# Kudo510/ImageSequenceRegistrationfor6DPoseEstimationLabeling

Measured on AMD Instinct MI355X. Metric: registered images/sec (T-LESS obj 1-like, synthetic) + final Chamfer error, higher is better.
Workload: dtype bf16

## Files before the change

### imagesequenceregistrationfor6dposeestimationlabeling_amd/_capi.py

```python
from __future__ import annotations

import ctypes as C
from pathlib import Path

import torch

import os

_PKG = Path(__file__).resolve().parent
LIB_PATH = Path(os.environ["ISR_HIP_LIB"]) if os.environ.get("ISR_HIP_LIB") else _PKG / "libisr_hip.so"

ISR_OK = 0
ABI_VERSION = 6
DTYPE_BF16 = 0
DTYPE_F32 = 1
DTYPE_BF16_LOG2 = 2
DTYPE_BF16_LOG2_SCREENED = 3
RANSAC_STAGED = 0
RANSAC_SEQUENTIAL = 1
INLIERS_REFIT = 0
INLIERS_RANSAC = 1
FINAL_REFIT = 0
FINAL_EPNP = 1
TUNE = {"nn_path": 0, "nn_filter": 1, "icp_warm": 2, "nn_plan_rq": 3, "nn_plan_blocks": 4,
        "nn_tile_st": 5, "nn_tile_sq": 6, "nn_tile_tb": 7, "ep_wsum_valu": 8, "k1_f32_chain": 9, "k1_split": 10}


class IsrError(RuntimeError):
    pass


_lib = None

_vp = C.c_void_p
_i = C.c_int
_sz = C.c_size_t
_d = C.c_double
_f = C.c_float
_u64 = C.c_uint64
_i64 = C.c_int64
# ... 185 lines not shown

SAMPLE_GRAD_SIGNATURES = {
    "isr_sample_grad_workspace_bytes": (_sz, [_i, _i, _i, _i]),
    "isr_sample_nearest_backward": (_i, [_vp, _i, _i, _i, _i, _vp, _i, _vp, _vp, _sz, _vp]),
    "isr_sample_nearest_backward_host": (_i, [_vp, _i, _i, _i, _i, _vp, _i, _vp]),
    "isr_sample_grad_geometry": (_i, [_i]),
}

EA_GRAD_SIGNATURES = {
    "isr_ea_march_backward": (_i, [_vp, _vp, _i, _i, _i, _f, _vp, _vp, _vp, _vp, _vp]),
    "isr_ea_march_backward_host": (_i, [_vp, _vp, _i, _i, _i, _f, _vp, _vp, _vp, _vp]),
    "isr_ea_grad_geometry": (_i, [_i]),
    "isr_ea_grad_rays_per_group": (_i, [_i]),
}

MC_SIGNATURES = {
    "isr_mc_workspace_bytes": (_sz, [_i, _i, _i]),
    "isr_mc_count": (_i, [_vp, _i, _i, _i, _f, _vp, _vp, _sz, _vp]),
    "isr_mc_emit": (_i, [_vp, _i, _i, _i, _f, _vp, _sz, _vp, _i64, _vp, _i64, _vp]),
    "isr_mc_count_host": (_i, [_vp, _i, _i, _i, _f, _vp]),
    "isr_mc_emit_host": (_i, [_vp, _i, _i, _i, _f, _vp, _i64, _vp, _i64]),
}


def lib() -> C.CDLL:
    global _lib
    if _lib is not None:
        return _lib
    if not LIB_PATH.exists():
        raise IsrError(
            f"{LIB_PATH} is missing: build it with "
            "`python -m imagesequenceregistrationfor6dposeestimationlabeling_amd.build` "
            "(there is no CPU fallback)")
    try:
        L = C.CDLL(str(LIB_PATH))
    except OSError as e:
        raise IsrError(f"cannot load {LIB_PATH}: {e}") from e
    for name, (res, args) in {**SIGNATURES, **FIELD_SIGNATURES, **FPS_SIGNATURES, **DENSITY_SIGNATURES,
                               **DENSITY_DIR_SIGNATURES, **RADIUS_SIGNATURES, **MC_SIGNATURES, **KNN_SIGNATURES,
                               **RAYS_SIGNATURES, **RADIANCE_SIGNATURES, **RESAMPLE_SIGNATURES,
                               **CONTRASTIVE_SIGNATURES, **FIELD_GRAD_SIGNATURES, **SAMPLE_GRAD_SIGNATURES,
                               **EA_GRAD_SIGNATURES}.items():
        try:
            fn = getattr(L, name)
        except AttributeError as e:
            raise IsrError(f"{LIB_PATH} does not export {name}") from e
        fn.restype = res
        fn.argtypes = args
    if L.isr_abi_version() != ABI_VERSION:
        raise IsrError(f"ABI version {L.isr_abi_version()} != {ABI_VERSION}")
    _lib = L
    return L


def check(rc: int, what: str) -> None:
    if rc != ISR_OK:
        msg = lib().isr_last_error()
# ... 30 lines not shown
```

### imagesequenceregistrationfor6dposeestimationlabeling_amd/csrc/capi_common.hip

```cpp
#include "isr_common.hpp"

#include <atomic>
#include <cstdlib>
#include <cstring>

namespace isr {

char* last_error_buf() {
  static thread_local char buf[512] = {0};
  return buf;
}

void set_error(const char* fmt, ...) {
  va_list ap;
  va_start(ap, fmt);
  vsnprintf(last_error_buf(), 512, fmt, ap);
  va_end(ap);
}

namespace {

struct Tuning {
  std::atomic<int> v[ISR_TUNE_COUNT];
  Tuning() {
    const int defaults[ISR_TUNE_COUNT] = {-1, -1, 1, 0, 0, 0, 0, 0, 0, 0, 0};
    for (int i = 0; i < ISR_TUNE_COUNT; ++i) v[i].store(defaults[i], std::memory_order_relaxed);
    if (const char* e = getenv("ISR_NN_GRID")) { if (e[0] >= '0' && e[0] <= '2') v[ISR_TUNE_NN_PATH] = e[0] - '0'; }
    if (const char* e = getenv("ISR_NN_FILTER")) { if (e[0] == '0' || e[0] == '1') v[ISR_TUNE_NN_FILTER] = e[0] - '0'; }
    if (const char* e = getenv("ISR_ICP_WARM")) { if (e[0] == '0') v[ISR_TUNE_ICP_WARM] = 0; }
    if (const char* e = getenv("ISR_NN_PLAN")) {
      int rq = 0; long want = 0;
      if (sscanf(e, "%d,%ld", &rq, &want) >= 1) {
        if (rq == 1 || rq == 4) v[ISR_TUNE_NN_PLAN_RQ] = rq;
        if (want > 0) v[ISR_TUNE_NN_PLAN_BLOCKS] = (int)want;
      }
    }
    if (const char* e = getenv("ISR_NN_TILE")) {
      double st = 0, sq = 0; int tb = 0;
      (void)sscanf(e, "%lf,%lf,%d", &st, &sq, &tb);
      if (st > 0) v[ISR_TUNE_NN_TILE_ST] = (int)(st * 1000.0 + 0.5);
      if (sq > 0) v[ISR_TUNE_NN_TILE_SQ] = (int)(sq * 1000.0 + 0.5);
      if (tb > 0) v[ISR_TUNE_NN_TILE_TB] = tb;
    }
  }
// ... 93 lines not shown
```

### imagesequenceregistrationfor6dposeestimationlabeling_amd/csrc/nn_batched.hip

```cpp
#include "isr_common.hpp"

#include <cstddef>
#include <cstdlib>

namespace {

#ifndef ISR_NN_PACKED_BATCH
#define ISR_NN_PACKED_BATCH 1
#endif
constexpr int kThreads = 256;
constexpr int kTile = 256;
constexpr int kGroup = 8;
constexpr int kNV = 18;

__device__ __forceinline__ void xform64(const double* __restrict__ T, float x, float y, float z,
                                        double& ox, double& oy, double& oz) {
  if (T == nullptr) {
    ox = x; oy = y; oz = z;
    return;
  }
  const double dx = x, dy = y, dz = z;
  ox = fma(T[2], dz, fma(T[1], dy, fma(T[0], dx, T[3])));
  oy = fma(T[6], dz, fma(T[5], dy, fma(T[4], dx, T[7])));
  oz = fma(T[10], dz, fma(T[9], dy, fma(T[8], dx, T[11])));
// ... 22 lines not shown
      v[3 + a] = fmaxf(v[3 + a], __shfl_xor(v[3 + a], o, 64));
    }
  }
  if ((threadIdx.x & 63) == 0) {
#pragma unroll
    for (int a = 0; a < 6; ++a) red[a][threadIdx.x >> 6] = v[a];
  }
  __syncthreads();
  if (threadIdx.x < 6) {
    const int a = threadIdx.x;
    const float r0 = red[a][0], r1 = red[a][1], r2 = red[a][2], r3 = red[a][3];
    box[6 * (size_t)blockIdx.x + a] = a < 3 ? fminf(fminf(r0, r1), fminf(r2, r3)) : fmaxf(fmaxf(r0, r1), fmaxf(r2, r3));
  }
}

constexpr int kIcpItemDoubles = 20;
constexpr int kIcpStateInts = 8;
template <int RQ, bool FILTER, bool EXACT = false, bool CULL = false, bool ITEMS = false>
__global__ __launch_bounds__(kThreads) void nn_search_kernel(
    const float* __restrict__ qry, int Nq, const float* __restrict__ tgt, int Nt,
    const double* __restrict__ Tq, const double* __restrict__ Tt, int split_len, int nsplit,
    float* __restrict__ part_d2, int32_t* __restrict__ part_idx, const int32_t* __restrict__ skip,
    const int32_t* __restrict__ unresolved, unsigned long long* __restrict__ packed = nullptr,
    const int32_t* __restrict__ warm = nullptr, int32_t* __restrict__ amb = nullptr,
    const float* __restrict__ t2_bound = nullptr, const float* __restrict__ tile_box = nullptr, float cull_r2 = 0.f,
    size_t qry_item_stride = 0) {
  __shared__ __attribute__((aligned(16))) float lds[2][FILTER ? 4 : 3][kTile];
  __shared__ float tile_t2[2][kThreads / 64];
  if (ITEMS) {
    if (skip[(size_t)blockIdx.z * kIcpStateInts]) return;
    qry += (size_t)blockIdx.z * qry_item_stride;
  } else if (skip && *skip) {
    return;
  }
  if (unresolved && *unresolved == 0) return;

  const int tid = threadIdx.x;
  const int b = blockIdx.z;
  const int split = blockIdx.y;
  if (unresolved) {
    int mine = 0;
#pragma unroll
    for (int r = 0; r < RQ; ++r) {
// ... 28 lines not shown
    const int w = warm ? warm[(size_t)b * Nq + qi] : -1;
    widx[r] = (w >= 0 && w < Nt) ? w : -1;
    if (w >= 0 && w < Nt) {
      double tx, ty, tz;
      xform64(tt, tgt[3 * (size_t)w], tgt[3 * (size_t)w + 1], tgt[3 * (size_t)w + 2], tx, ty, tz);
      const float dx = qx[r] - (float)tx, dy = qy[r] - (float)ty, dz = qz[r] - (float)tz;
      best[r] = __builtin_fmaf(dz, dz, __builtin_fmaf(dy, dy, dx * dx));
      bidx[r] = w;
    }
    if (EXACT) {
      dlt[r] = 1.001f * kU0 * (__builtin_sqrtf(q2[r]) + __builtin_sqrtf(*t2_bound));
      thx[r] = nearthr(r, best[r]);
      am[r] = false;
    }
  }

  const int t0 = split * split_len;
  const int t1 = min(Nt, t0 + split_len);
  const int ntiles = (t1 - t0 + kTile - 1) / kTile;
  constexpr float kU = 5.9604645e-8f;

  float wlo[3], whi[3], wb = __builtin_inff();
  if (CULL && tile_box) {
    float b = 0.f;
    wlo[0] = wlo[1] = wlo[2] = 3.0e38f; whi[0] = whi[1] = whi[2] = -3.0e38f;
#pragma unroll
    for (int r = 0; r < RQ; ++r) {
      float br = EXACT ? thx[r] : best[r];
      if (cull_r2 > 0.f) br = fminf(br, cull_r2);
      b = fmaxf(b, br);
      wlo[0] = fminf(wlo[0], qx[r]); wlo[1] = fminf(wlo[1], qy[r]); wlo[2] = fminf(wlo[2], qz[r]);
      whi[0] = fmaxf(whi[0], qx[r]); whi[1] = fmaxf(whi[1], qy[r]); whi[2] = fmaxf(whi[2], qz[r]);
    }
#pragma unroll
    for (int o = 32; o >= 1; o >>= 1) {
      b = fmaxf(b, __shfl_xor(b, o, 64));
#pragma unroll
      for (int a = 0; a < 3; ++a) {
        wlo[a] = fminf(wlo[a], __shfl_xor(wlo[a], o, 64));
        whi[a] = fmaxf(whi[a], __shfl_xor(whi[a], o, 64));
      }
    }
    wb = __uint_as_float(__builtin_amdgcn_readfirstlane(__float_as_uint(__builtin_fmaf(b, 1.0001f, 1.0e-4f))));
#pragma unroll
    for (int a = 0; a < 3; ++a) {
      wlo[a] = __uint_as_float(__builtin_amdgcn_readfirstlane(__float_as_uint(wlo[a])));
      whi[a] = __uint_as_float(__builtin_amdgcn_readfirstlane(__float_as_uint(whi[a])));
    }
  }
  auto tile_culled = [&](int tile) {
    if (!CULL || !tile_box) return false;
    const float* bx = tile_box + 6 * (size_t)(t0 / kTile + tile);
    float d2 = 0.f;
#pragma unroll
    for (int a = 0; a < 3; ++a) {
      const float g = fmaxf(0.f, fmaxf(wlo[a] - bx[3 + a], bx[a] - whi[a]));
      d2 = __builtin_fmaf(g, g, d2);
    }
    return d2 > wb;
  };
  if (CULL && tile_box && ntiles == 1) {
    if (!__syncthreads_or(tile_culled(0) ? 0 : 1)) return;
  }

  auto stage = [&](int tile, int buf) {
    const int j = t0 + tile * kTile + tid;
    if (!FILTER) {
      float x = 3.0e38f, y = 3.0e38f, z = 3.0e38f;
      if (j < t1) {
        double dx, dy, dz;
        xform64(tt, tgt[3 * (size_t)j], tgt[3 * (size_t)j + 1], tgt[3 * (size_t)j + 2], dx, dy, dz);
        x = (float)dx; y = (float)dy; z = (float)dz;
      }
      lds[buf][0][tid] = x;
      lds[buf][1][tid] = y;
      lds[buf][2][tid] = z;
      return;
    }
    float x = 0.f, y = 0.f, z = 0.f, t2 = 3.0e38f, t2m = 0.f;
    if (j < t1) {
      double dx, dy, dz;
// ... 9 lines not shown
#pragma unroll
    for (int o = 32; o >= 1; o >>= 1) t2m = fmaxf(t2m, __shfl_xor(t2m, o, 64));
    if ((tid & 63) == 0) tile_t2[buf][tid >> 6] = t2m;
  };
  auto threshold = [&](int r, float t2max) {
    return __builtin_fmaf(64.f * kU, q2[r] + t2max, __builtin_fmaf(EXACT ? thx[r] : best[r], 1.f + 8.f * kU, -q2[r]));
  };

  if (ntiles > 0) stage(0, 0);
  __syncthreads();
  for (int tile = 0; tile < ntiles; ++tile) {
    const int buf = tile & 1;
    if (tile + 1 < ntiles) stage(tile + 1, buf ^ 1);
    const int jbase = t0 + tile * kTile;
    if (__builtin_amdgcn_readfirstlane(tile_culled(tile) ? 1 : 0) != 0) {
      __syncthreads();
      continue;
    }
    if (!FILTER) {
#pragma unroll 2
      for (int g = 0; g < kTile; g += kGroup) {
        float tx[kGroup], ty[kGroup], tz[kGroup];
#pragma unroll
        for (int v = 0; v < kGroup; v += 4) {
          const float4 a = *reinterpret_cast<const float4*>(&lds[buf][0][g + v]);
          const float4 c = *reinterpret_cast<const float4*>(&lds[buf][1][g + v]);
          const float4 e = *reinterpret_cast<const float4*>(&lds[buf][2][g + v]);
          tx[v] = a.x; tx[v + 1] = a.y; tx[v + 2] = a.z; tx[v + 3] = a.w;
          ty[v] = c.x; ty[v + 1] = c.y; ty[v + 2] = c.z; ty[v + 3] = c.w;
          tz[v] = e.x; tz[v + 1] = e.y; tz[v + 2] = e.z; tz[v + 3] = e.w;
// ... 21 lines not shown
              thx[r] = nearthr(r, best[r]);
              bool t = (bidx0 >= 0) & (bidx0 != bidx[r]) & (best0 <= thx[r]);
#pragma unroll
              for (int v = 0; v < kGroup; ++v) t |= (d[v] <= thx[r]) & (d[v] < 2.9e38f) & (jbase + g + v != bidx[r]);
              am[r] |= t;
            }
          }
        }
      }
      __syncthreads();
      continue;
    }
    const float t2max = fmaxf(fmaxf(tile_t2[buf][0], tile_t2[buf][1]), fmaxf(tile_t2[buf][2], tile_t2[buf][3]));
#pragma unroll
    for (int r = 0; r < RQ; ++r) thr[r] = threshold(r, t2max);
#pragma unroll 2
    for (int g = 0; g < kTile; g += kGroup) {
      float tx[kGroup], ty[kGroup], tz[kGroup], tw[kGroup];
#pragma unroll
      for (int v = 0; v < kGroup; v += 4) {
        const float4 a = *reinterpret_cast<const float4*>(&lds[buf][0][g + v]);
        const float4 c = *reinterpret_cast<const float4*>(&lds[buf][1][g + v]);
        const float4 e = *reinterpret_cast<const float4*>(&lds[buf][2][g + v]);
        const float4 w = *reinterpret_cast<const float4*>(&lds[buf][FILTER ? 3 : 0][g + v]);
        tx[v] = a.x; tx[v + 1] = a.y; tx[v + 2] = a.z; tx[v + 3] = a.w;
        ty[v] = c.x; ty[v + 1] = c.y; ty[v + 2] = c.z; ty[v + 3] = c.w;
        tz[v] = e.x; tz[v + 1] = e.y; tz[v + 2] = e.z; tz[v + 3] = e.w;
        tw[v] = w.x; tw[v + 1] = w.y; tw[v + 2] = w.z; tw[v + 3] = w.w;
      }
#pragma unroll
      for (int r = 0; r < RQ; ++r) {
        float sc[kGroup];
// ... 22 lines not shown
            }
          }
          if (EXACT) {
            thx[r] = nearthr(r, best[r]);
            bool t = (bidx0 >= 0) & (bidx0 != bidx[r]) & (best0 <= thx[r]);
#pragma unroll
            for (int v = 0; v < kGroup; ++v) t |= (dd[v] <= thx[r]) & (jbase + g + v != bidx[r]);
            am[r] |= t;
          }
          thr[r] = threshold(r, t2max);
        }
      }
    }
    __syncthreads();
  }

  if (packed) {
    unsigned long long old[RQ];
    bool posted[RQ];
#pragma unroll
    for (int r = 0; r < RQ; ++r) {
      const int qi = query_of<RQ>(r);
      const bool own = widx[r] < 0 || bidx[r] != widx[r] || (widx[r] >= t0 && widx[r] < t1);
      posted[r] = qi < Nq && bidx[r] >= 0 && own;
      old[r] = ~0ull;
      if (posted[r]) {
        const unsigned long long mine = ((unsigned long long)__float_as_uint(best[r]) << 32) | (unsigned int)bidx[r];
        if (EXACT) old[r] = atomicMin(&packed[(size_t)b * Nq + qi], mine);
        else atomicMin(&packed[(size_t)b * Nq + qi], mine);
      }
// ... 196 lines not shown
  }
  double lam = A[0][0];
#pragma unroll
  for (int k = 0; k < 4; ++k) q[k] = V[k][0];
#pragma unroll
  for (int j = 1; j < 4; ++j) {
    if (A[j][j] > lam) {
      lam = A[j][j];
#pragma unroll
      for (int k = 0; k < 4; ++k) q[k] = V[k][j];
    }
  }
}

constexpr int kIcpLanes = 16;

__device__ void icp_reduce_and_update(const double* __restrict__ part_sums, int nblk, int Ns, int max_iter,
                                      double rel_fitness, double rel_rmse, double* __restrict__ T,
                                      IcpState* __restrict__ st, double* __restrict__ result) {
  __shared__ double part[kNV][kIcpLanes];
  __shared__ double v[kNV];
  for (int idx = threadIdx.x; idx < kNV * kIcpLanes; idx += blockDim.x) {
    const int k = idx / kIcpLanes, l = idx % kIcpLanes;
    double s = 0.0;
    for (int i = l; i < nblk; i += kIcpLanes) s += part_sums[(size_t)i * kNV + k];
    part[k][l] = s;
  }
  __syncthreads();
  if (threadIdx.x < kNV) {
    double s = 0.0;
// ... 221 lines not shown
  }
  const size_t per_b = (size_t)p.nsplit * Nq * 8;
  long bc = (long)(kPartBudget / (per_b ? per_b : 1));
  if (bc < 1) bc = 1;
  if (bc > B) bc = B;
  if (bc > 65535) bc = 65535;
  p.bchunk = (int)bc;
  return p;
}

constexpr int kFilterMinTiles = 4;
void launch_search(const NNPlan& p, const dim3& grid, hipStream_t stream, const float* qry, int Nq, const float* tgt, int Nt,
                   const double* tq, const double* tt, float* part_d2, int32_t* part_idx, const int32_t* skip,
                   const int32_t* unresolved, unsigned long long* packed, const int32_t* warm, int32_t* amb = nullptr,
                   const float* t2_bound = nullptr, const float* tile_box = nullptr, float cull_r2 = 0.f,
                   bool items = false, size_t qry_item_stride = 0) {
  bool filter = warm != nullptr || p.split_len >= kFilterMinTiles * kTile;
  if (const int f = isr::tuning(ISR_TUNE_NN_FILTER); f >= 0 && !warm) filter = f == 1;
#define ISR_SEARCH(RQv, Fv)                                                                                              \
  nn_search_kernel<RQv, Fv><<<grid, kThreads, 0, stream>>>(qry, Nq, tgt, Nt, tq, tt, p.split_len, p.nsplit, part_d2, part_idx, \
                                                           skip, unresolved, packed, warm)
#define ISR_SEARCH_X(RQv, Fv)                                                                                            \
  nn_search_kernel<RQv, Fv, true, Fv><<<grid, kThreads, 0, stream>>>(qry, Nq, tgt, Nt, tq, tt, p.split_len, p.nsplit, part_d2, \
                                                                     part_idx, skip, unresolved, packed, warm, amb, t2_bound, tile_box, cull_r2)
#define ISR_SEARCH_ITEMS(RQv, Fv)                                                                                        \
  nn_search_kernel<RQv, Fv, true, Fv, true><<<grid, kThreads, 0, stream>>>(qry, Nq, tgt, Nt, tq, tt, p.split_len, p.nsplit,    \
                                                                           part_d2, part_idx, skip, unresolved, packed, warm, \
                                                                           amb, t2_bound, tile_box, cull_r2, qry_item_stride)
  if (items) {
    if (p.rq == 4) { if (filter) ISR_SEARCH_ITEMS(4, true); else ISR_SEARCH_ITEMS(4, false); }
    else { if (filter) ISR_SEARCH_ITEMS(1, true); else ISR_SEARCH_ITEMS(1, false); }
    return;
  }
  if (amb) {
    if (p.rq == 4) { if (filter) ISR_SEARCH_X(4, true); else ISR_SEARCH_X(4, false); }
    else { if (filter) ISR_SEARCH_X(1, true); else ISR_SEARCH_X(1, false); }
    return;
  }
  if (p.rq == 4) { if (filter) ISR_SEARCH(4, true); else ISR_SEARCH(4, false); }
  else { if (filter) ISR_SEARCH(1, true); else ISR_SEARCH(1, false); }
#undef ISR_SEARCH_ITEMS
#undef ISR_SEARCH_X
#undef ISR_SEARCH
}

}

extern "C" size_t isr_nn_batched_workspace_bytes(int Nq, int Nt, int B) {
  if (Nq <= 0 || Nt <= 0 || B <= 0) return 0;
  const NNPlan p = make_plan(Nq, Nt, B);
  size_t n = 0;
  n += isr::align_up((size_t)p.bchunk * p.nsplit * Nq * sizeof(float), 256);
  n += isr::align_up((size_t)p.bchunk * p.nsplit * Nq * sizeof(int32_t), 256);
  n += isr::align_up((size_t)B * p.fblocks * kNV * sizeof(double), 256);
  if (p.grid) n += grid_ws_bytes(Nt);
  if (p.tile) n += tile_ws_bytes(Nq, Nt);
  return n + 256;
}

// ... 75 lines not shown
}

extern "C" int isr_add_metric(const float* verts, int V, const double* Ta, const double* Tb, int B,
                              double* mean_out, isr_stream_t stream) {
  ISR_REQUIRE(verts && mean_out, "isr_add_metric: null pointer");
  ISR_REQUIRE(V > 0 && B > 0, "isr_add_metric: V=%d B=%d", V, B);
  add_metric_kernel<<<B, kThreads, 0, isr::as_stream(stream)>>>(verts, V, Ta, Tb, mean_out);
  ISR_CHECK_LAUNCH("add_metric_kernel");
  return ISR_OK;
}

extern "C" size_t isr_icp_workspace_bytes(int Ns, int Nt) {
  if (Ns <= 0 || Nt <= 0) return 0;
  const NNPlan p = make_plan(Ns, Nt, 1, true);
  return isr::align_up((size_t)p.fblocks * kNV * sizeof(double), 256) + isr::align_up((size_t)Ns * 8, 256) +
         2 * isr::align_up((size_t)Ns * 4, 256) + isr::align_up((size_t)((Nt + kTile - 1) / kTile) * 6 * sizeof(float), 256) + 2048;
}

extern "C" int isr_icp_point_to_point(const float* src, int Ns, const float* tgt, int Nt, double threshold,
                                      int max_iter, double rel_fitness, double rel_rmse, double* T_io,
                                      double* result, void* ws, size_t ws_bytes, isr_stream_t stream_) {
  ISR_REQUIRE(src && tgt && T_io && result, "isr_icp_point_to_point: null pointer");
  ISR_REQUIRE(Ns > 0 && Nt > 0 && max_iter >= 0 && threshold > 0, "isr_icp_point_to_point: Ns=%d Nt=%d max_iter=%d", Ns, Nt, max_iter);
  if (!ws || ws_bytes < isr_icp_workspace_bytes(Ns, Nt)) {
    isr::set_error("isr_icp_point_to_point: workspace %zu < %zu", ws_bytes, isr_icp_workspace_bytes(Ns, Nt));
    return ISR_ERR_WORKSPACE;
  }
  hipStream_t stream = isr::as_stream(stream_);
  const NNPlan p = make_plan(Ns, Nt, 1, true);
  isr::Workspace w(ws, ws_bytes);
  double* part_sums = w.take<double>((size_t)p.fblocks * kNV);
  IcpState* st = w.take<IcpState>(1);
  unsigned long long* packed = w.take<unsigned long long>(Ns);
  int32_t* prev_idx = w.take<int32_t>(Ns);
  int32_t* amb = w.take<int32_t>(Ns);
  float* t2_bound = w.take<float>(1);
  float* tile_box = w.take<float>((size_t)((Nt + kTile - 1) / kTile) * 6);
  const bool warm = isr::tuning(ISR_TUNE_ICP_WARM) != 0;
  icp_init_kernel<<<(Ns + kThreads - 1) / kThreads, kThreads, 0, stream>>>(st, T_io, packed, amb, Ns);
  cloud_r2max_kernel<<<1, kThreads, 0, stream>>>(tgt, Nt, t2_bound);
#ifndef ISR_ICP_CULL
#define ISR_ICP_CULL 1
#endif
  const float cull_r2 = (float)(threshold * threshold * 1.0001 + 1e-6);
  if (ISR_ICP_CULL) tile_box_kernel<<<(Nt + kTile - 1) / kTile, 256, 0, stream>>>(tgt, Nt, tile_box);
  const dim3 grid(p.qblocks, p.nsplit, 1);
  for (int it = 0; it <= max_iter; ++it) {
    const int32_t* w_idx = (it > 0 && warm) ? prev_idx : nullptr;
    launch_search(p, grid, stream, src, Ns, tgt, Nt, T_io, nullptr, nullptr, nullptr, &st->done, nullptr, packed, w_idx, amb,
                  t2_bound, ISR_ICP_CULL ? tile_box : nullptr, cull_r2);
    icp_finalize_update_kernel<<<p.fblocks, kThreads, 0, stream>>>(src, Ns, tgt, Nt, threshold, packed, prev_idx, amb, part_sums,
                                                                   max_iter, rel_fitness, rel_rmse, T_io, st, result);
  }
  ISR_CHECK_LAUNCH("icp kernels");
  return ISR_OK;
}

extern "C" size_t isr_icp_point_to_point_batch_workspace_bytes(int Ns, int Nt, int B) {
  if (Ns <= 0 || Nt <= 0 || B <= 0) return 0;
  const NNPlan p = make_plan(Ns, Nt, B, true);
  return isr::align_up((size_t)B * p.fblocks * kNV * sizeof(double), 256) + isr::align_up((size_t)B * sizeof(IcpState), 256) +
         isr::align_up((size_t)B * Ns * 8, 256) + 2 * isr::align_up((size_t)B * Ns * 4, 256) +
         isr::align_up((size_t)((Nt + kTile - 1) / kTile) * 6 * sizeof(float), 256) + 2048;
}

extern "C" int isr_icp_point_to_point_batch(const float* src, size_t src_item_stride, int Ns, const float* tgt, int Nt, int B,
                                            double threshold, int max_iter, double rel_fitness, double rel_rmse,
                                            double* state, void* ws, size_t ws_bytes, isr_stream_t stream_) {
  ISR_REQUIRE(src && tgt && state, "isr_icp_point_to_point_batch: null pointer");
  ISR_REQUIRE(Ns > 0 && Nt > 0 && B >= 0 && B <= 65535, "isr_icp_point_to_point_batch: Ns=%d Nt=%d must be positive, B=%d in [0, 65535]",
              Ns, Nt, B);
  ISR_REQUIRE(threshold > 0 && max_iter >= 0, "isr_icp_point_to_point_batch: threshold=%g must be positive, max_iter=%d non-negative",
              threshold, max_iter);
  ISR_REQUIRE(src_item_stride == 0 || src_item_stride >= 3 * (size_t)Ns,
              "isr_icp_point_to_point_batch: src_item_stride=%zu must be 0 (one source for all items) or at least 3*Ns=%zu floats",
              src_item_stride, 3 * (size_t)Ns);
  if (B == 0) return ISR_OK;
  if (!ws || ws_bytes < isr_icp_point_to_point_batch_workspace_bytes(Ns, Nt, B)) {
    isr::set_error("isr_icp_point_to_point_batch: workspace %zu < %zu", ws_bytes,
                   isr_icp_point_to_point_batch_workspace_bytes(Ns, Nt, B));
    return ISR_ERR_WORKSPACE;
  }
  hipStream_t stream = isr::as_stream(stream_);
  const NNPlan p = make_plan(Ns, Nt, B, true);
  isr::Workspace w(ws, ws_bytes);
  double* part_sums = w.take<double>((size_t)B * p.fblocks * kNV);
  IcpState* st = w.take<IcpState>(B);
  unsigned long long* packed = w.take<unsigned long long>((size_t)B * Ns);
  int32_t* prev_idx = w.take<int32_t>((size_t)B * Ns);
  int32_t* amb = w.take<int32_t>((size_t)B * Ns);
  float* t2_bound = w.take<float>(1);
  float* tile_box = w.take<float>((size_t)((Nt + kTile - 1) / kTile) * 6);
  const bool warm = isr::tuning(ISR_TUNE_ICP_WARM) != 0;
  icp_init_kernel<<<dim3((Ns + kThreads - 1) / kThreads, B), kThreads, 0, stream>>>(st, state, packed, amb, Ns, kIcpItemDoubles);
  cloud_r2max_kernel<<<1, kThreads, 0, stream>>>(tgt, Nt, t2_bound);
  const float cull_r2 = (float)(threshold * threshold * 1.0001 + 1e-6);
  if (ISR_ICP_CULL) tile_box_kernel<<<(Nt + kTile - 1) / kTile, 256, 0, stream>>>(tgt, Nt, tile_box);
  const dim3 grid(p.qblocks, p.nsplit, B);
  for (int it = 0; it <= max_iter; ++it) {
    const int32_t* w_idx = (it > 0 && warm) ? prev_idx : nullptr;
    launch_search(p, grid, stream, src, Ns, tgt, Nt, state, nullptr, nullptr, nullptr, &st->done, nullptr, packed, w_idx, amb,
                  t2_bound, ISR_ICP_CULL ? tile_box : nullptr, cull_r2, true, src_item_stride);
    icp_finalize_update_kernel<<<dim3(p.fblocks, B), kThreads, 0, stream>>>(src, Ns, tgt, Nt, threshold, packed, prev_idx, amb,
                                                                             part_sums, max_iter, rel_fitness, rel_rmse, state,
                                                                             st, state + 16, src_item_stride, kIcpItemDoubles);
  }
  ISR_CHECK_LAUNCH("icp batch kernels");
  return ISR_OK;
}
```

### imagesequenceregistrationfor6dposeestimationlabeling_amd/ops.py

```python
from __future__ import annotations

import ctypes
from dataclasses import dataclass

import numpy as np

import torch

from . import _capi
from ._capi import check, current_stream, lib, ptr, require_cuda

_workspaces: dict[tuple, torch.Tensor] = {}

_timers: dict[str, list] | None = None


def enable_timing(on: bool = True) -> None:
    global _timers
    _timers = {} if on else None


def drain_timing() -> dict[str, tuple[int, float, float]]:
    out = {}
    if _timers is None:
# ... 34 lines not shown
        self.old = {k: L.isr_tuning_get(k) for k in self.knobs}
        for k, v in self.knobs.items():
            check(L.isr_tuning_set(k, v), "isr_tuning_set")
        return self

    def __exit__(self, *exc):
        L = lib()
        for k, v in self.old.items():
            L.isr_tuning_set(k, v)
        return False


def set_tuning(**knobs) -> None:
    for k, v in knobs.items():
        check(lib().isr_tuning_set(_capi.TUNE[k], int(v)), "isr_tuning_set")


def set_tile_plan(plan: str | None) -> None:
    if plan is None:
        set_tuning(nn_tile_st=0, nn_tile_sq=0, nn_tile_tb=0)
    else:
        st, sq, tb = plan.split(",")
        set_tuning(nn_tile_st=round(float(st) * 1000), nn_tile_sq=round(float(sq) * 1000), nn_tile_tb=int(tb))


def workspace(device: torch.device, nbytes: int, tag: str = "default") -> torch.Tensor:
    key = (device.index, torch.cuda.current_stream(device).cuda_stream, tag)
    buf = _workspaces.get(key)
    if buf is not None and buf.numel() >= nbytes:
        return buf
# ... 1874 lines not shown
```

### include/isr_hip.h

```cpp
#ifndef ISR_HIP_H
#define ISR_HIP_H

#include <stddef.h>
#include <stdint.h>

#ifdef __cplusplus
extern "C" {
#endif

#define ISR_ABI_VERSION 6

#define ISR_OK 0
#define ISR_ERR_ARG (-1)
#define ISR_ERR_WORKSPACE (-2)
#define ISR_ERR_HIP (-3)
#define ISR_ERR_UNSUPPORTED (-4)

#define ISR_DTYPE_BF16 0
#define ISR_DTYPE_F32 1
#define ISR_DTYPE_BF16_LOG2 2

#define ISR_DTYPE_BF16_LOG2_SCREENED 3

typedef void* isr_stream_t;
// ... 1 lines not shown
int isr_abi_version(void);
const char* isr_last_error(void);
int isr_device_count(void);

#define ISR_TUNE_NN_PATH 0
#define ISR_TUNE_NN_FILTER 1
#define ISR_TUNE_ICP_WARM 2
#define ISR_TUNE_NN_PLAN_RQ 3
#define ISR_TUNE_NN_PLAN_BLOCKS 4
#define ISR_TUNE_NN_TILE_ST 5
#define ISR_TUNE_NN_TILE_SQ 6
#define ISR_TUNE_NN_TILE_TB 7
#define ISR_TUNE_EP_WSUM_VALU 8
#define ISR_TUNE_K1_F32_CHAIN 9
#define ISR_TUNE_K1_SPLIT 10
#define ISR_TUNE_COUNT 11
int isr_tuning_set(int knob, int value);
int isr_tuning_get(int knob);

size_t isr_corr_argmax_workspace_bytes(int P, int N, int D, int dtype);
int isr_corr_argmax(const void* Q, const void* K, int P, int N, int D, int ldq, int ldk, int dtype,
                    int32_t* idx, float* logp, float* lse, void* ws, size_t ws_bytes,
                    isr_stream_t stream);

int isr_corr_argmax_digits(const void* Q, const void* K, int P, int N, int D, int ldq, int ldk, int dtype,
                           int32_t* idx, float* logp, float* lse, int rows_per_image, const int32_t* n_rows,
                           int32_t* digit_hist, void* ws, size_t ws_bytes, isr_stream_t stream);

int isr_corr_argmax_phase(const void* Q, const void* K, int P, int N, int D, int ldq, int ldk, int dtype,
                          int32_t* idx, float* logp, float* lse, int rows_per_image, const int32_t* n_rows,
                          int32_t* digit_hist, int phase, void* ws, size_t ws_bytes, isr_stream_t stream);
// ... 196 lines not shown
```

Before: 1119.

## Add per-group bounding-sphere culling inside ICP nearest-neighbour tile search

Builds a per-8-point bounding-sphere table for each target tile, plus a per-tile compactness flag. In the filtered ICP NN search kernel, each wave tests its query bounds against each group sphere and skips distance evaluation for groups that cannot improve the best match. The aim is to cut the inner-loop distance arithmetic on compact tiles, at the cost of an extra table kernel, extra LDS staging, and a per-tile bound test. Optional counters and host reference functions are added for diagnostics, and the cull is on by default.

```diff
diff --git a/imagesequenceregistrationfor6dposeestimationlabeling_amd/_capi.py b/imagesequenceregistrationfor6dposeestimationlabeling_amd/_capi.py
--- a/imagesequenceregistrationfor6dposeestimationlabeling_amd/_capi.py
+++ b/imagesequenceregistrationfor6dposeestimationlabeling_amd/_capi.py
@@ -23,7 +23,8 @@
 FINAL_REFIT = 0
 FINAL_EPNP = 1
 TUNE = {"nn_path": 0, "nn_filter": 1, "icp_warm": 2, "nn_plan_rq": 3, "nn_plan_blocks": 4,
-        "nn_tile_st": 5, "nn_tile_sq": 6, "nn_tile_tb": 7, "ep_wsum_valu": 8, "k1_f32_chain": 9, "k1_split": 10}
+        "nn_tile_st": 5, "nn_tile_sq": 6, "nn_tile_tb": 7, "ep_wsum_valu": 8, "k1_f32_chain": 9, "k1_split": 10,
+        "icp_group_cull": 11}
 
 
 class IsrError(RuntimeError):
@@ -239,6 +240,12 @@
     "isr_ea_grad_rays_per_group": (_i, [_i]),
 }
 
+ICP_CULL_SIGNATURES = {
+    "isr_icp_group_cull_counter": (_i, [_vp]),
+    "isr_icp_group_table_host": (_i, [_vp, _i, _vp, _vp]),
+    "isr_icp_group_skip_host": (_i, [_vp, _vp, _i, _f, _vp, _vp]),
+}
+
 MC_SIGNATURES = {
     "isr_mc_workspace_bytes": (_sz, [_i, _i, _i]),
     "isr_mc_count": (_i, [_vp, _i, _i, _i, _f, _vp, _vp, _sz, _vp]),
@@ -265,7 +272,7 @@
                                **DENSITY_DIR_SIGNATURES, **RADIUS_SIGNATURES, **MC_SIGNATURES, **KNN_SIGNATURES,
                                **RAYS_SIGNATURES, **RADIANCE_SIGNATURES, **RESAMPLE_SIGNATURES,
                                **CONTRASTIVE_SIGNATURES, **FIELD_GRAD_SIGNATURES, **SAMPLE_GRAD_SIGNATURES,
-                               **EA_GRAD_SIGNATURES}.items():
+                               **EA_GRAD_SIGNATURES, **ICP_CULL_SIGNATURES}.items():
         try:
             fn = getattr(L, name)
         except AttributeError as e:
diff --git a/imagesequenceregistrationfor6dposeestimationlabeling_amd/csrc/capi_common.hip b/imagesequenceregistrationfor6dposeestimationlabeling_amd/csrc/capi_common.hip
--- a/imagesequenceregistrationfor6dposeestimationlabeling_amd/csrc/capi_common.hip
+++ b/imagesequenceregistrationfor6dposeestimationlabeling_amd/csrc/capi_common.hip
@@ -23,11 +23,12 @@
 struct Tuning {
   std::atomic<int> v[ISR_TUNE_COUNT];
   Tuning() {
-    const int defaults[ISR_TUNE_COUNT] = {-1, -1, 1, 0, 0, 0, 0, 0, 0, 0, 0};
+    const int defaults[ISR_TUNE_COUNT] = {-1, -1, 1, 0, 0, 0, 0, 0, 0, 0, 0, 1};
     for (int i = 0; i < ISR_TUNE_COUNT; ++i) v[i].store(defaults[i], std::memory_order_relaxed);
     if (const char* e = getenv("ISR_NN_GRID")) { if (e[0] >= '0' && e[0] <= '2') v[ISR_TUNE_NN_PATH] = e[0] - '0'; }
     if (const char* e = getenv("ISR_NN_FILTER")) { if (e[0] == '0' || e[0] == '1') v[ISR_TUNE_NN_FILTER] = e[0] - '0'; }
     if (const char* e = getenv("ISR_ICP_WARM")) { if (e[0] == '0') v[ISR_TUNE_ICP_WARM] = 0; }
+    if (const char* e = getenv("ISR_ICP_GROUP_CULL")) { if (e[0] >= '0' && e[0] <= '2') v[ISR_TUNE_ICP_GROUP_CULL] = e[0] - '0'; }
     if (const char* e = getenv("ISR_NN_PLAN")) {
       int rq = 0; long want = 0;
       if (sscanf(e, "%d,%ld", &rq, &want) >= 1) {
diff --git a/imagesequenceregistrationfor6dposeestimationlabeling_amd/csrc/nn_batched.hip b/imagesequenceregistrationfor6dposeestimationlabeling_amd/csrc/nn_batched.hip
--- a/imagesequenceregistrationfor6dposeestimationlabeling_amd/csrc/nn_batched.hip
+++ b/imagesequenceregistrationfor6dposeestimationlabeling_amd/csrc/nn_batched.hip
@@ -1,9 +1,13 @@
 #include "isr_common.hpp"
-
+#include "nn_group_cull.hpp"
+
+#include <atomic>
 #include <cstddef>
 #include <cstdlib>
 
 namespace {
+
+namespace gcull = isr::gcull;
 
 #ifndef ISR_NN_PACKED_BATCH
 #define ISR_NN_PACKED_BATCH 1
@@ -60,9 +64,80 @@
   }
 }
 
+__global__ __launch_bounds__(256) void group_sphere_kernel(const float* __restrict__ tgt, int Nt, float* __restrict__ tab,
+                                                           int32_t* __restrict__ tile_ok, int force) {
+  __shared__ float red[8][4];
+  const int tid = threadIdx.x, lane = tid & 63;
+  const int j = blockIdx.x * 256 + tid;
+  const bool valid = j < Nt;
+  float t[3] = {0.f, 0.f, 0.f}, lo[3], hi[3];
+#pragma unroll
+  for (int a = 0; a < 3; ++a) {
+    if (valid) t[a] = tgt[3 * (size_t)j + a];
+    lo[a] = valid ? t[a] : 3.0e38f;
+    hi[a] = valid ? t[a] : -3.0e38f;
+  }
+  int n = valid ? 1 : 0;
+#pragma unroll
+  for (int o = 1; o < gcull::kGroupRows; o <<= 1) {
+#pragma unroll
+    for (int a = 0; a < 3; ++a) {
+      lo[a] = fminf(lo[a], __shfl_xor(lo[a], o, 64));
+      hi[a] = fmaxf(hi[a], __shfl_xor(hi[a], o, 64));
+    }
+    n += __shfl_xor(n, o, 64);
+  }
+  float c[3];
+  gcull::centre(lo, hi, c);
+  float d2 = valid ? gcull::dist2(c, t[0], t[1], t[2]) : 0.f;
+#pragma unroll
+  for (int o = 1; o < gcull::kGroupRows; o <<= 1) d2 = fmaxf(d2, __shfl_xor(d2, o, 64));
+  float e[gcull::kEntryFloats];
+  gcull::entry(c, d2, n, e);
+  if ((tid & (gcull::kGroupRows - 1)) == 0) {
+    float* o = tab + gcull::kEntryFloats * ((size_t)blockIdx.x * 32 + (tid >> 3));
+    *reinterpret_cast<float4*>(o) = make_float4(e[0], e[1], e[2], e[3]);
+    *reinterpret_cast<float4*>(o + 4) = make_float4(e[4], 0.f, 0.f, 0.f);
+  }
+  const float rg = n > 0 ? e[4] : 0.f;
+  float s = 0.f;
+  int ng = 0;
+#pragma unroll
+  for (int g = 0; g < 8; ++g) {
+    s += __shfl(rg, 8 * g, 64);
+    ng += __shfl(n, 8 * g, 64) > 0 ? 1 : 0;
+  }
+#pragma unroll
+  for (int o = 8; o <= 32; o <<= 1) {
+#pragma unroll
+    for (int a = 0; a < 3; ++a) {
+      lo[a] = fminf(lo[a], __shfl_xor(lo[a], o, 64));
+      hi[a] = fmaxf(hi[a], __shfl_xor(hi[a], o, 64));
+    }
+  }
+  if (lane == 0) {
+#pragma unroll
+    for (int a = 0; a < 3; ++a) { red[a][tid >> 6] = lo[a]; red[3 + a][tid >> 6] = hi[a]; }
+    red[6][tid >> 6] = s;
+    red[7][tid >> 6] = (float)ng;
+  }
+  __syncthreads();
+  if (tid == 0) {
+    float ex[3];
+#pragma unroll
+    for (int a = 0; a < 3; ++a)
+      ex[a] = fmaxf(fmaxf(red[3 + a][0], red[3 + a][1]), fmaxf(red[3 + a][2], red[3 + a][3])) -
+              fminf(fminf(red[a][0], red[a][1]), fminf(red[a][2], red[a][3]));
+    const float sum = ((red[6][0] + red[6][1]) + red[6][2]) + red[6][3];
+    const int ngt = (int)(((red[7][0] + red[7][1]) + red[7][2]) + red[7][3]);
+    const float hd = 0.5f * __builtin_sqrtf(__builtin_fmaf(ex[2], ex[2], __builtin_fmaf(ex[1], ex[1], ex[0] * ex[0])));
+    tile_ok[blockIdx.x] = (force || gcull::tile_compact(sum, ngt, hd)) ? 1 : 0;
+  }
+}
+
 constexpr int kIcpItemDoubles = 20;
 constexpr int kIcpStateInts = 8;
-template <int RQ, bool FILTER, bool EXACT = false, bool CULL = false, bool ITEMS = false>
+template <int RQ, bool FILTER, bool EXACT = false, bool CULL = false, bool ITEMS = false, bool COUNT = false>
 __global__ __launch_bounds__(kThreads) void nn_search_kernel(
     const float* __restrict__ qry, int Nq, const float* __restrict__ tgt, int Nt,
     const double* __restrict__ Tq, const double* __restrict__ Tt, int split_len, int nsplit,
@@ -70,9 +145,15 @@
     const int32_t* __restrict__ unresolved, unsigned long long* __restrict__ packed = nullptr,
     const int32_t* __restrict__ warm = nullptr, int32_t* __restrict__ amb = nullptr,
     const float* __restrict__ t2_bound = nullptr, const float* __restrict__ tile_box = nullptr, float cull_r2 = 0.f,
-    size_t qry_item_stride = 0) {
+    size_t qry_item_stride = 0, const float* __restrict__ grp_tab = nullptr, const int32_t* __restrict__ grp_ok = nullptr,
+    unsigned long long* __restrict__ grp_count = nullptr) {
   __shared__ __attribute__((aligned(16))) float lds[2][FILTER ? 4 : 3][kTile];
   __shared__ float tile_t2[2][kThreads / 64];
+  constexpr bool GRP = FILTER && CULL;
+  constexpr bool CNT = GRP && COUNT;
+  __shared__ float4 grp_c[2][kTile / kGroup];
+  __shared__ float grp_r[2][kTile / kGroup];
+  __shared__ unsigned int grp_n[3];
   if (ITEMS) {
     if (skip[(size_t)blockIdx.z * kIcpStateInts]) return;
     qry += (size_t)blockIdx.z * qry_item_stride;
@@ -131,13 +212,26 @@
       am[r] = false;
     }
   }
+  const bool grp = GRP && grp_tab != nullptr && tile_box != nullptr;
+  if (CNT) {
+    if (tid < 3) grp_n[tid] = 0;
+    __syncthreads();
+  }
+  auto grp_note = [&](int k, int n) {
+    if ((tid & 63) == 0) atomicAdd(&grp_n[k], (unsigned)n);
+  };
+  auto grp_flush = [&]() {
+    if (!CNT) return;
+    __syncthreads();
+    if (tid < 3) atomicAdd(&grp_count[tid], (unsigned long long)grp_n[tid]);
+  };
 
   const int t0 = split * split_len;
   const int t1 = min(Nt, t0 + split_len);
   const int ntiles = (t1 - t0 + kTile - 1) / kTile;
   constexpr float kU = 5.9604645e-8f;
 
-  float wlo[3], whi[3], wb = __builtin_inff();
+  float wlo[3], whi[3], wb = __builtin_inff(), hW = 0.f;
   if (CULL && tile_box) {
     float b = 0.f;
     wlo[0] = wlo[1] = wlo[2] = 3.0e38f; whi[0] = whi[1] = whi[2] = -3.0e38f;
@@ -159,6 +253,7 @@
       }
     }
     wb = __uint_as_float(__builtin_amdgcn_readfirstlane(__float_as_uint(__builtin_fmaf(b, 1.0001f, 1.0e-4f))));
+    if (GRP && grp) hW = __uint_as_float(__builtin_amdgcn_readfirstlane(__float_as_uint(gcull::wave_cross(b))));
 #pragma unroll
     for (int a = 0; a < 3; ++a) {
       wlo[a] = __uint_as_float(__builtin_amdgcn_readfirstlane(__float_as_uint(wlo[a])));
@@ -177,11 +272,20 @@
     return d2 > wb;
   };
   if (CULL && tile_box && ntiles == 1) {
-    if (!__syncthreads_or(tile_culled(0) ? 0 : 1)) return;
+    if (!__syncthreads_or(tile_culled(0) ? 0 : 1)) {
+      if (CNT) grp_note(2, (t1 - t0 + kGroup - 1) / kGroup);
+      grp_flush();
+      return;
+    }
   }
 
   auto stage = [&](int tile, int buf) {
     const int j = t0 + tile * kTile + tid;
+    if (GRP && grp && tid < kTile / kGroup) {
+      const float* e = grp_tab + gcull::kEntryFloats * ((size_t)(t0 / kTile + tile) * (kTile / kGroup) + tid);
+      grp_c[buf][tid] = *reinterpret_cast<const float4*>(e);
+      grp_r[buf][tid] = e[4];
+    }
     if (!FILTER) {
       float x = 3.0e38f, y = 3.0e38f, z = 3.0e38f;
       if (j < t1) {
@@ -221,6 +325,7 @@
     if (tile + 1 < ntiles) stage(tile + 1, buf ^ 1);
     const int jbase = t0 + tile * kTile;
     if (__builtin_amdgcn_readfirstlane(tile_culled(tile) ? 1 : 0) != 0) {
+      if (CNT) grp_note(2, min(kTile / kGroup, (t1 - jbase + kGroup - 1) / kGroup));
       __syncthreads();
       continue;
     }
@@ -272,8 +377,35 @@
     const float t2max = fmaxf(fmaxf(tile_t2[buf][0], tile_t2[buf][1]), fmaxf(tile_t2[buf][2], tile_t2[buf][3]));
 #pragma unroll
     for (int r = 0; r < RQ; ++r) thr[r] = threshold(r, t2max);
+    unsigned int need = ~0u;
+    if (GRP && grp && __builtin_amdgcn_readfirstlane(grp_ok[t0 / kTile + tile]) != 0) {
+      float ngb[RQ];
+#pragma unroll
+      for (int r = 0; r < RQ; ++r) {
+        float br = EXACT ? thx[r] : best[r];
+        if (cull_r2 > 0.f) br = fminf(br, cull_r2);
+        ngb[r] = gcull::lane_bound(br, q2[r]);
+      }
+      need = 0u;
+#pragma unroll 4
+      for (int gi = 0; gi < kTile / kGroup; ++gi) {
+        const float4 cg = grp_c[buf][gi];
+        const float kw = gcull::rhs(cg.w, grp_r[buf][gi], hW);
+        float m = gcull::chain(qx[0], qy[0], qz[0], ngb[0], cg.x, cg.y, cg.z);
+#pragma unroll
+        for (int r = 1; r < RQ; ++r) m = fminf(m, gcull::chain(qx[r], qy[r], qz[r], ngb[r], cg.x, cg.y, cg.z));
+        need |= __any(!(m > kw)) ? (1u << gi) : 0u;
+      }
+    }
+    if (CNT) {
+      const int nv = min(kTile / kGroup, (t1 - jbase + kGroup - 1) / kGroup);
+      const int ev = __builtin_popcount(need & (nv < 32 ? (1u << nv) - 1u : ~0u));
+      grp_note(0, ev);
+      grp_note(1, nv - ev);
+    }
 #pragma unroll 2
     for (int g = 0; g < kTile; g += kGroup) {
+      if (GRP && !((need >> (g / kGroup)) & 1u)) continue;
       float tx[kGroup], ty[kGroup], tz[kGroup], tw[kGroup];
 #pragma unroll
       for (int v = 0; v < kGroup; v += 4) {
@@ -326,6 +458,7 @@
     }
     __syncthreads();
   }
+  grp_flush();
 
   if (packed) {
     unsigned long long old[RQ];
@@ -552,6 +685,10 @@
 }
 
 constexpr int kIcpLanes = 16;
+
+#ifndef ISR_ICP_CULL
+#define ISR_ICP_CULL 1
+#endif
 
 __device__ void icp_reduce_and_update(const double* __restrict__ part_sums, int nblk, int Ns, int max_iter,
                                       double rel_fitness, double rel_rmse, double* __restrict__ T,
@@ -803,7 +940,8 @@
                    const double* tq, const double* tt, float* part_d2, int32_t* part_idx, const int32_t* skip,
                    const int32_t* unresolved, unsigned long long* packed, const int32_t* warm, int32_t* amb = nullptr,
                    const float* t2_bound = nullptr, const float* tile_box = nullptr, float cull_r2 = 0.f,
-                   bool items = false, size_t qry_item_stride = 0) {
+                   bool items = false, size_t qry_item_stride = 0, const float* grp_tab = nullptr, const int32_t* grp_ok = nullptr,
+                   unsigned long long* grp_count = nullptr) {
   bool filter = warm != nullptr || p.split_len >= kFilterMinTiles * kTile;
   if (const int f = isr::tuning(ISR_TUNE_NN_FILTER); f >= 0 && !warm) filter = f == 1;
 #define ISR_SEARCH(RQv, Fv)                                                                                              \
@@ -811,11 +949,25 @@
                                                            skip, unresolved, packed, warm)
 #define ISR_SEARCH_X(RQv, Fv)                                                                                            \
   nn_search_kernel<RQv, Fv, true, Fv><<<grid, kThreads, 0, stream>>>(qry, Nq, tgt, Nt, tq, tt, p.split_len, p.nsplit, part_d2, \
-                                                                     part_idx, skip, unresolved, packed, warm, amb, t2_bound, tile_box, cull_r2)
+                                                                     part_idx, skip, unresolved, packed, warm, amb, t2_bound, tile_box, cull_r2, \
+                                                                     0, grp_tab, grp_ok, grp_count)
 #define ISR_SEARCH_ITEMS(RQv, Fv)                                                                                        \
   nn_search_kernel<RQv, Fv, true, Fv, true><<<grid, kThreads, 0, stream>>>(qry, Nq, tgt, Nt, tq, tt, p.split_len, p.nsplit,    \
                                                                            part_d2, part_idx, skip, unresolved, packed, warm, \
-                                                                           amb, t2_bound, tile_box, cull_r2, qry_item_stride)
+                                                                           amb, t2_bound, tile_box, cull_r2, qry_item_stride, grp_tab, grp_ok, \
+                                                                           grp_count)
+#define ISR_SEARCH_COUNT(RQv, ITv)                                                                                       \
+  nn_search_kernel<RQv, true, true, true, ITv, true><<<grid, kThreads, 0, stream>>>(qry, Nq, tgt, Nt, tq, tt, p.split_len,     \
+                                                                                     p.nsplit, part_d2, part_idx, skip,       \
+                                                                                     unresolved, packed, warm, amb, t2_bound, \
+                                                                                     tile_box, cull_r2, qry_item_stride,      \
+                                                                                     grp_tab, grp_ok, grp_count)
+  if (amb && filter && grp_count) {
+    if (items) { if (p.rq == 4) ISR_SEARCH_COUNT(4, true); else ISR_SEARCH_COUNT(1, true); }
+    else { if (p.rq == 4) ISR_SEARCH_COUNT(4, false); else ISR_SEARCH_COUNT(1, false); }
+    return;
+  }
+#undef ISR_SEARCH_COUNT
   if (items) {
     if (p.rq == 4) { if (filter) ISR_SEARCH_ITEMS(4, true); else ISR_SEARCH_ITEMS(4, false); }
     else { if (filter) ISR_SEARCH_ITEMS(1, true); else ISR_SEARCH_ITEMS(1, false); }
@@ -832,6 +984,13 @@
 #undef ISR_SEARCH_X
 #undef ISR_SEARCH
 }
+
+size_t group_table_bytes(int Nt) {
+  const size_t ntiles = (size_t)((Nt + kTile - 1) / kTile);
+  return isr::align_up(ntiles * (kTile / kGroup) * gcull::kEntryFloats * sizeof(float), 256) + isr::align_up(ntiles * sizeof(int32_t), 256);
+}
+
+std::atomic<unsigned long long*> g_group_counter{nullptr};
 
 }
 
@@ -937,7 +1096,7 @@
   if (Ns <= 0 || Nt <= 0) return 0;
   const NNPlan p = make_plan(Ns, Nt, 1, true);
   return isr::align_up((size_t)p.fblocks * kNV * sizeof(double), 256) + isr::align_up((size_t)Ns * 8, 256) +
-         2 * isr::align_up((size_t)Ns * 4, 256) + isr::align_up((size_t)((Nt + kTile - 1) / kTile) * 6 * sizeof(float), 256) + 2048;
+         2 * isr::align_up((size_t)Ns * 4, 256) + isr::align_up((size_t)((Nt + kTile - 1) / kTile) * 6 * sizeof(float), 256) + group_table_bytes(Nt) + 2048;
 }
 
 extern "C" int isr_icp_point_to_point(const float* src, int Ns, const float* tgt, int Nt, double threshold,
@@ -959,19 +1118,21 @@
   int32_t* amb = w.take<int32_t>(Ns);
   float* t2_bound = w.take<float>(1);
   float* tile_box = w.take<float>((size_t)((Nt + kTile - 1) / kTile) * 6);
+  float* grp_tab = w.take<float>((size_t)((Nt + kTile - 1) / kTile) * (kTile / kGroup) * gcull::kEntryFloats);
+  int32_t* grp_ok = w.take<int32_t>((size_t)((Nt + kTile - 1) / kTile));
   const bool warm = isr::tuning(ISR_TUNE_ICP_WARM) != 0;
+  const int gmode = ISR_ICP_CULL ? isr::tuning(ISR_TUNE_ICP_GROUP_CULL) : 0;
+  unsigned long long* const grp_count = g_group_counter.load(std::memory_order_relaxed);
   icp_init_kernel<<<(Ns + kThreads - 1) / kThreads, kThreads, 0, stream>>>(st, T_io, packed, amb, Ns);
   cloud_r2max_kernel<<<1, kThreads, 0, stream>>>(tgt, Nt, t2_bound);
-#ifndef ISR_ICP_CULL
-#define ISR_ICP_CULL 1
-#endif
   const float cull_r2 = (float)(threshold * threshold * 1.0001 + 1e-6);
   if (ISR_ICP_CULL) tile_box_kernel<<<(Nt + kTile - 1) / kTile, 256, 0, stream>>>(tgt, Nt, tile_box);
+  if (gmode) group_sphere_kernel<<<(Nt + kTile - 1) / kTile, 256, 0, stream>>>(tgt, Nt, grp_tab, grp_ok, gmode == 2);
   const dim3 grid(p.qblocks, p.nsplit, 1);
   for (int it = 0; it <= max_iter; ++it) {
     const int32_t* w_idx = (it > 0 && warm) ? prev_idx : nullptr;
     launch_search(p, grid, stream, src, Ns, tgt, Nt, T_io, nullptr, nullptr, nullptr, &st->done, nullptr, packed, w_idx, amb,
-                  t2_bound, ISR_ICP_CULL ? tile_box : nullptr, cull_r2);
+                  t2_bound, ISR_ICP_CULL ? tile_box : nullptr, cull_r2, false, 0, gmode ? grp_tab : nullptr, grp_ok, grp_count);
     icp_finalize_update_kernel<<<p.fblocks, kThreads, 0, stream>>>(src, Ns, tgt, Nt, threshold, packed, prev_idx, amb, part_sums,
                                                                    max_iter, rel_fitness, rel_rmse, T_io, st, result);
   }
@@ -984,7 +1145,7 @@
   const NNPlan p = make_plan(Ns, Nt, B, true);
   return isr::align_up((size_t)B * p.fblocks * kNV * sizeof(double), 256) + isr::align_up((size_t)B * sizeof(IcpState), 256) +
          isr::align_up((size_t)B * Ns * 8, 256) + 2 * isr::align_up((size_t)B * Ns * 4, 256) +
-         isr::align_up((size_t)((Nt + kTile - 1) / kTile) * 6 * sizeof(float), 256) + 2048;
+         isr::align_up((size_t)((Nt + kTile - 1) / kTile) * 6 * sizeof(float), 256) + group_table_bytes(Nt) + 2048;
 }
 
 extern "C" int isr_icp_point_to_point_batch(const float* src, size_t src_item_stride, int Ns, const float* tgt, int Nt, int B,
@@ -1014,16 +1175,21 @@
   int32_t* amb = w.take<int32_t>((size_t)B * Ns);
   float* t2_bound = w.take<float>(1);
   float* tile_box = w.take<float>((size_t)((Nt + kTile - 1) / kTile) * 6);
+  float* grp_tab = w.take<float>((size_t)((Nt + kTile - 1) / kTile) * (kTile / kGroup) * gcull::kEntryFloats);
+  int32_t* grp_ok = w.take<int32_t>((size_t)((Nt + kTile - 1) / kTile));
   const bool warm = isr::tuning(ISR_TUNE_ICP_WARM) != 0;
+  const int gmode = ISR_ICP_CULL ? isr::tuning(ISR_TUNE_ICP_GROUP_CULL) : 0;
+  unsigned long long* const grp_count = g_group_counter.load(std::memory_order_relaxed);
   icp_init_kernel<<<dim3((Ns + kThreads - 1) / kThreads, B), kThreads, 0, stream>>>(st, state, packed, amb, Ns, kIcpItemDoubles);
   cloud_r2max_kernel<<<1, kThreads, 0, stream>>>(tgt, Nt, t2_bound);
   const float cull_r2 = (float)(threshold * threshold * 1.0001 + 1e-6);
   if (ISR_ICP_CULL) tile_box_kernel<<<(Nt + kTile - 1) / kTile, 256, 0, stream>>>(tgt, Nt, tile_box);
+  if (gmode) group_sphere_kernel<<<(Nt + kTile - 1) / kTile, 256, 0, stream>>>(tgt, Nt, grp_tab, grp_ok, gmode == 2);
   const dim3 grid(p.qblocks, p.nsplit, B);
   for (int it = 0; it <= max_iter; ++it) {
     const int32_t* w_idx = (it > 0 && warm) ? prev_idx : nullptr;
     launch_search(p, grid, stream, src, Ns, tgt, Nt, state, nullptr, nullptr, nullptr, &st->done, nullptr, packed, w_idx, amb,
-                  t2_bound, ISR_ICP_CULL ? tile_box : nullptr, cull_r2, true, src_item_stride);
+                  t2_bound, ISR_ICP_CULL ? tile_box : nullptr, cull_r2, true, src_item_stride, gmode ? grp_tab : nullptr, grp_ok, grp_count);
     icp_finalize_update_kernel<<<dim3(p.fblocks, B), kThreads, 0, stream>>>(src, Ns, tgt, Nt, threshold, packed, prev_idx, amb,
                                                                              part_sums, max_iter, rel_fitness, rel_rmse, state,
                                                                              st, state + 16, src_item_stride, kIcpItemDoubles);
@@ -1031,3 +1197,25 @@
   ISR_CHECK_LAUNCH("icp batch kernels");
   return ISR_OK;
 }
+
+extern "C" int isr_icp_group_cull_counter(unsigned long long* counts) {
+  g_group_counter.store(counts, std::memory_order_relaxed);
+  return ISR_OK;
+}
+
+extern "C" int isr_icp_group_table_host(const float* tgt, int Nt, float* tab, int32_t* tile_ok) {
+  ISR_REQUIRE(tgt && tab && tile_ok && Nt > 0, "isr_icp_group_table_host: null pointer or Nt=%d", Nt);
+  gcull::table_host(tgt, Nt, tab, tile_ok);
+  return ISR_OK;
+}
+
+extern "C" int isr_icp_group_skip_host(const float* q, const float* bound, int n, float bmax, const float* entry, int32_t* skip) {
+  ISR_REQUIRE(q && bound && entry && skip && n >= 0, "isr_icp_group_skip_host: null pointer or n=%d", n);
+  const float hW = gcull::wave_cross(bmax);
+  for (int i = 0; i < n; ++i) {
+    const float qx = q[3 * (size_t)i], qy = q[3 * (size_t)i + 1], qz = q[3 * (size_t)i + 2];
+    const float q2 = fmaf(qz, qz, fmaf(qy, qy, qx * qx));
+    skip[i] = gcull::chain(qx, qy, qz, gcull::lane_bound(bound[i], q2), entry[0], entry[1], entry[2]) > gcull::rhs(entry[3], entry[4], hW) ? 1 : 0;
+  }
+  return ISR_OK;
+}
diff --git a/imagesequenceregistrationfor6dposeestimationlabeling_amd/csrc/nn_group_cull.hpp b/imagesequenceregistrationfor6dposeestimationlabeling_amd/csrc/nn_group_cull.hpp
--- /dev/null
+++ b/imagesequenceregistrationfor6dposeestimationlabeling_amd/csrc/nn_group_cull.hpp
@@ -0,0 +1,90 @@
+#pragma once
+
+#include <math.h>
+
+#if defined(__HIPCC__)
+#define ISR_GC_HD __host__ __device__ __forceinline__
+#else
+#define ISR_GC_HD inline
+#endif
+
+namespace isr {
+namespace gcull {
+
+constexpr int kGroupRows = 8;
+constexpr int kEntryFloats = 8;
+constexpr float kU = 5.9604645e-8f;
+constexpr float kUp = 1.000002f;
+constexpr float kNoBound = 1.0e30f;
+constexpr float kEmptyKg = -3.0e38f;
+
+ISR_GC_HD float dist2(const float c[3], float tx, float ty, float tz) {
+  const float dx = c[0] - tx, dy = c[1] - ty, dz = c[2] - tz;
+  return fmaf(dz, dz, fmaf(dy, dy, dx * dx));
+}
+
+ISR_GC_HD void centre(const float lo[3], const float hi[3], float c[3]) {
+  for (int a = 0; a < 3; ++a) c[a] = 0.5f * lo[a] + 0.5f * hi[a];
+}
+
+ISR_GC_HD void entry(const float c[3], float d2max, int nrows, float e[kEntryFloats]) {
+  const float rg = kUp * sqrtf(d2max);
+  const float rg2 = rg * rg;
+  const float c2 = fmaf(c[2], c[2], fmaf(c[1], c[1], c[0] * c[0]));
+  e[0] = -2.f * c[0]; e[1] = -2.f * c[1]; e[2] = -2.f * c[2];
+  e[3] = nrows > 0 ? fmaf(64.f * kU, rg2 + c2, rg2 - c2) : kEmptyKg;
+  e[4] = rg;
+  e[5] = e[6] = e[7] = 0.f;
+}
+
+ISR_GC_HD float lane_bound(float b, float q2) {
+  b = fminf(b, kNoBound);
+  return q2 - fmaf(64.f * kU, b + q2, b);
+}
+
+ISR_GC_HD float wave_cross(float bmax) { return (2.f * kUp) * sqrtf(fminf(bmax, kNoBound)); }
+
+ISR_GC_HD float chain(float qx, float qy, float qz, float ngb, float m2cx, float m2cy, float m2cz) {
+  return fmaf(qx, m2cx, fmaf(qy, m2cy, fmaf(qz, m2cz, ngb)));
+}
+ISR_GC_HD float rhs(float kg, float rg, float hW) { return fmaf(rg, hW, kg); }
+
+ISR_GC_HD bool tile_compact(float sum_rg, int ngroups, float half_diag) { return sum_rg <= 0.5f * (float)ngroups * half_diag; }
+
+inline void table_host(const float* tgt, int Nt, float* tab, int* tile_ok) {
+  const int ntiles = (Nt + 255) / 256;
+  for (int t = 0; t < ntiles; ++t) {
+    float blo[3] = {3.0e38f, 3.0e38f, 3.0e38f}, bhi[3] = {-3.0e38f, -3.0e38f, -3.0e38f}, sum = 0.f;
+    int ng = 0;
+    float rgs[32];
+    for (int g = 0; g < 32; ++g) {
+      const int j0 = t * 256 + g * kGroupRows, n = Nt - j0 < 0 ? 0 : (Nt - j0 < kGroupRows ? Nt - j0 : kGroupRows);
+      float lo[3] = {3.0e38f, 3.0e38f, 3.0e38f}, hi[3] = {-3.0e38f, -3.0e38f, -3.0e38f}, c[3], d2 = 0.f;
+      for (int i = 0; i < n; ++i)
+        for (int a = 0; a < 3; ++a) {
+          lo[a] = fminf(lo[a], tgt[3 * (size_t)(j0 + i) + a]);
+          hi[a] = fmaxf(hi[a], tgt[3 * (size_t)(j0 + i) + a]);
+        }
+      centre(lo, hi, c);
+      for (int i = 0; i < n; ++i)
+        d2 = fmaxf(d2, dist2(c, tgt[3 * (size_t)(j0 + i)], tgt[3 * (size_t)(j0 + i) + 1], tgt[3 * (size_t)(j0 + i) + 2]));
+      float* e = tab + kEntryFloats * ((size_t)t * 32 + g);
+      entry(c, d2, n, e);
+      rgs[g] = n > 0 ? e[4] : 0.f;
+      if (n > 0) {
+        ++ng;
+        for (int a = 0; a < 3; ++a) { blo[a] = fminf(blo[a], lo[a]); bhi[a] = fmaxf(bhi[a], hi[a]); }
+      }
+    }
+    for (int w = 0; w < 4; ++w) {
+      float s = 0.f;
+      for (int g = 0; g < 8; ++g) s += rgs[8 * w + g];
+      sum = w == 0 ? s : sum + s;
+    }
+    const float ex = bhi[0] - blo[0], ey = bhi[1] - blo[1], ez = bhi[2] - blo[2];
+    tile_ok[t] = tile_compact(sum, ng, 0.5f * sqrtf(fmaf(ez, ez, fmaf(ey, ey, ex * ex)))) ? 1 : 0;
+  }
+}
+
+}
+}
diff --git a/imagesequenceregistrationfor6dposeestimationlabeling_amd/ops.py b/imagesequenceregistrationfor6dposeestimationlabeling_amd/ops.py
--- a/imagesequenceregistrationfor6dposeestimationlabeling_amd/ops.py
+++ b/imagesequenceregistrationfor6dposeestimationlabeling_amd/ops.py
@@ -72,6 +72,24 @@
 def set_tuning(**knobs) -> None:
     for k, v in knobs.items():
         check(lib().isr_tuning_set(_capi.TUNE[k], int(v)), "isr_tuning_set")
+
+
+class icp_group_cull_counts:
+
+    def __init__(self, device):
+        self.buf = torch.zeros(3, dtype=torch.int64, device=device)
+
+    def __enter__(self):
+        check(lib().isr_icp_group_cull_counter(self.buf.data_ptr()), "isr_icp_group_cull_counter")
+        return self
+
+    def read(self) -> tuple[int, int, int]:
+        return tuple(int(v) for v in self.buf.cpu().tolist())
+
+    def __exit__(self, *exc):
+        torch.cuda.synchronize(self.buf.device)
+        lib().isr_icp_group_cull_counter(None)
+        return False
 
 
 def set_tile_plan(plan: str | None) -> None:
diff --git a/include/isr_hip.h b/include/isr_hip.h
--- a/include/isr_hip.h
+++ b/include/isr_hip.h
@@ -39,7 +39,8 @@
 #define ISR_TUNE_EP_WSUM_VALU 8
 #define ISR_TUNE_K1_F32_CHAIN 9
 #define ISR_TUNE_K1_SPLIT 10
-#define ISR_TUNE_COUNT 11
+#define ISR_TUNE_ICP_GROUP_CULL 11
+#define ISR_TUNE_COUNT 12
 int isr_tuning_set(int knob, int value);
 int isr_tuning_get(int knob);
 
diff --git a/include/isr_icp_cull.h b/include/isr_icp_cull.h
--- /dev/null
+++ b/include/isr_icp_cull.h
@@ -0,0 +1,23 @@
+#ifndef ISR_ICP_CULL_H
+#define ISR_ICP_CULL_H
+
+#include <stddef.h>
+#include <stdint.h>
+
+#include "isr_hip.h"
+
+#ifdef __cplusplus
+extern "C" {
+#endif
+
+int isr_icp_group_cull_counter(unsigned long long* counts);
+
+int isr_icp_group_table_host(const float* tgt, int Nt, float* tab, int32_t* tile_ok);
+
+int isr_icp_group_skip_host(const float* q, const float* bound, int n, float bmax, const float* entry, int32_t* skip);
+
+#ifdef __cplusplus
+}
+#endif
+
+#endif
```

Result: no change. 1125, median of 6 (+0.6%).
